# neobotix/neo_mpc_planner2

Measured on AMD Instinct MI355X. Metric: MPC solves/sec (control_steps=3, 500x500 costmap), higher is better.
Workload: dtype f64

## Files before the change

### neo_mpc_planner2_amd/csrc/adjoint.h

```cpp
#pragma once
#include "neo_mpc_device.h"
#include "wave_ops.h"
#include "fast_math.h"
#include "solver_context.h"
#include "costmap.h"
#include "riccati.h"

namespace neo_mpc {
namespace {

template <bool kTame, bool kRiccati, int kFew = 0>
__device__ __forceinline__ void adjoint_by_scans(const SolveArgs& a, const Ctx& c, double* L, bool exact_step, int lane, int n,
                                                 bool& free_path, int& nhops) {
  auto scan = [](double v) { if constexpr (kFew > 0) return wave_scan_few<kFew>(v); else return wave_scan(v); };
  constexpr int kLast = kFew > 0 ? kFew - 1 : 63;
  const DevParams& p = a.p;
  const double* u = L + a.lds.u;
  double* gs = L + a.lds.gs;
  float* RS = reinterpret_cast<float*>(L + a.lds.ric);
  float* ARTF = reinterpret_cast<float*>(L + a.lds.rt);
  const bool on = lane < n;
  const double vx = on ? u[3 * lane] : 0.0, vy = on ? u[3 * lane + 1] : 0.0, w = on ? u[3 * lane + 2] : 0.0;
  const double th = scan(w * p.dt);
  double sn, cs;
  sincos_heading<kTame>(th, &sn, &cs);
  const double ddx = (vx * cs - vy * sn) * p.dt, ddy = (vx * sn + vy * cs) * p.dt;
  const double x = scan(ddx), y = scan(ddy);
  double rt = on ? -2.0 * p.wo_n * (c.tyaw - th) : 0.0;
  if (lane == n - 1) rt += -2.0 * p.wterm_o * (c.fyaw - th);
  const double rx = on ? -2.0 * p.wt_n * (c.cx - x) : 0.0, ry = on ? -2.0 * p.wt_n * (c.cy - y) : 0.0;
  const double px = scan(rx), py = scan(ry);
  const double SX = lane_value(px, kLast) - px + rx, SY = lane_value(py, kLast) - py + ry;
  const double tt = on ? rt - ddy * SX + ddx * SY : 0.0;
  const double pt = scan(tt);
  const double ST = lane_value(pt, kLast) - pt + tt;
  int raw_here = 0;
  bool has_hop = false;
  float hop_x = 0.0f, hop_y = 0.0f;
  if (on) {
    gs[3 * lane] = p.dt * (cs * SX + sn * SY);
    gs[3 * lane + 1] = p.dt * (-sn * SX + cs * SY);
    gs[3 * lane + 2] = p.dt * ST;
    if (kRiccati) {
      float* rs = RS + kRicStage * lane;
      rs[RS_CS] = (float)cs; rs[RS_SN] = (float)sn; rs[RS_PX] = (float)ddx; rs[RS_PY] = (float)ddy;
      double wxx, wxy, wyy, wlx, wly;
      raw_here = edge_stickiness(a, c, L, x, y, cs, sn, wxx, wxy, wyy, wlx, wly, has_hop, hop_x, hop_y);
      rs[RS_WXX] = (float)wxx; rs[RS_WXY] = (float)wxy; rs[RS_WYY] = (float)wyy;
      rs[RS_WLX] = (float)wlx; rs[RS_WLY] = (float)wly;
      rs[RS_SY] = exact_step ? (float)SY : 0.0f;
      ARTF[2 * lane + 1] = exact_step ? (float)SX : 0.0f;
    }
  }
  if (kRiccati) {
    free_path = __ballot(raw_here != 0) == 0ull;
    const unsigned long long hmask = __ballot(has_hop);
    const int rank = __popcll(hmask & ((1ull << lane) - 1ull));
    double* t = L + a.lds.tol;
    if (has_hop && rank < kHopLanes) {
      reinterpret_cast<int*>(t + T_HOP_STAGE)[rank] = lane;
      reinterpret_cast<float*>(t + T_HOP_VEC)[2 * rank] = hop_x;
      reinterpret_cast<float*>(t + T_HOP_VEC)[2 * rank + 1] = hop_y;
    }
    nhops = min(__popcll(hmask), (int)kHopLanes);
    if (lane == 0) reinterpret_cast<int*>(t + T_HOP_STAGE)[kHopLanes] = nhops;
  }
  WAVE_SYNC();
}

template <int kSteps, bool kTame>
__device__ __forceinline__ void adjoint_short_sweep(const SolveArgs& a, const Ctx& c, double* L, bool have_trig, int lane, int n) {
  const DevParams& p = a.p;
  const double* u = L + a.lds.u;
  double* gs = L + a.lds.gs;
  double* ACS = L + a.lds.cs;
  double* ASN = L + a.lds.sn;
  double* ADX = L + a.lds.dxs;
  double* ADY = L + a.lds.dys;
  double* ARX = L + a.lds.rx;
  double* ARY = L + a.lds.ry;
// ... 36 lines not shown
```

### neo_mpc_planner2_amd/csrc/k1_solve.h

```cpp
#pragma once
#include <hip/hip_runtime.h>
#include <hip/hip_ext.h>
#include <math.h>
#include <stdint.h>
#include <stdlib.h>

#include "neo_mpc_device.h"
#include "wave_ops.h"
#include "fast_math.h"
#include "solver_context.h"
#include "solver_rules.h"
#include "costmap.h"
#include "feasible_set.h"
#include "rollout.h"
#include "riccati.h"
#include "adjoint.h"
#include "tangent_cone.h"
#include "dense_newton.h"
#include "lbfgs.h"
#include "cell_scan.h"
#include "k1_timing.h"

namespace neo_mpc {
namespace {

constexpr int kStallIterations = NEO_RULE_STALL_ITERATIONS;
constexpr int kBlockedRun = NEO_RULE_BLOCKED_RUN;
constexpr double kBlockedStep = NEO_RULE_BLOCKED_STEP;
constexpr double kFinalFracGaussNewton = NEO_RULE_FINAL_FRAC_GN;
// ... 143 lines not shown
  }
  s.flags = flags; s.cold = cold;
  return true;
}

template <int kMinWavesPerSimd, int kSteps, int kDir, bool kTame, int kStaticTile, int kLayoutSteps, bool kRouted = false>
__device__ __forceinline__ bool solve_search(double* L, uint32_t b, SolveCarry& sc) {
  constexpr bool kCovered = kStaticTile > 0;
  constexpr bool kNewton = kDir == 1;
  constexpr bool kRiccati = kDir == 2;
  constexpr bool kSecond = kDir != 0;
  constexpr bool kBlockedRule = kNewton || kRouted;
  static_assert(!kRiccati || kSteps == 0 || kRouted, "the stage-wise direction: run-time-sized, or the routed kernel's control_steps-3 branch");
  static_assert(!kRouted || (kRiccati && kSteps == kRoutedSteps), "the routed branch is the stage-wise one, three stages in registers");
  constexpr int kFew = (kRiccati && kSteps > 0) ? kSteps : 0;
  constexpr int kNwSteps = !kNewton ? 1 : kSteps ? kSteps : kNewtonMaxSteps;
  constexpr bool kVectorPose = kTame;
  constexpr int kRegSteps = kSteps ? kSteps : 1;
  constexpr int kPairs = kSteps ? 4 : NEO_MPC_MAX_LBFGS_MEMORY;
  double f = sc.f;
  const bool cold = sc.cold;
  int npairs = 0, head = 0, nfev = sc.nfev, it = sc.it, status = sc.status, stall = 0;
  int blocked_run = 0;
  int nblocked = 1;
  double u_term = 0.0;
  double gain1 = INFINITY, gain2 = INFINITY;
  bool final_step = false;
  double alpha = 1.0;
  bool scanned = false;
  int nscans = 0;
// ... 35 lines not shown
    if (kRouted && lane == 0) L[a.lds.tol + T_KINK] = p.kink_radius_stagewise;
    alpha = kRiccati ? fmax(1.0, n * 0.125) : 1.0;
    if (kFew && lane == 0) { double* t = L + a.lds.tol; t[T_GAIN1] = INFINITY; t[T_GAIN2] = INFINITY; t[T_ALPHA] = alpha; }
    if (kRiccati && lane == 0) L[a.lds.tol + T_MU] = n > 8 ? (double)(n - 8) * 0.125 : 0.0;
  }
  bool v_feasible = false;
  if (kRiccati) {
    double b0 = c.v0, b1 = c.v1, b2 = c.v2;
    asm volatile("" : "+v"(b0), "+v"(b1), "+v"(b2));
    project_block<kTame>(p, b0, b1, b2);
    v_feasible = b0 == c.v0 && b1 == c.v1 && b2 == c.v2;
  }
  double my_scale;
  {
    int l0 = lane_again();
    my_scale = kRiccati ? 0.0 : lane_scale<kSecond>(l0);
  }
  for (; it < p.max_it && !scan_only; ++it) {
    int lane = lane_again();
    const bool exact_step = kRiccati && nblocked == 0;
    int tol_off = a.lds.tol;
    asm volatile("" : "+s"(tol_off));
    const double* TOL = L + tol_off;
    NEO_PHASE_DECL;
    NEO_PHASE(0);
    constexpr int kVars = 3 * kNwSteps;
    const int nvr = kSteps ? kVars : nv;
    bool free_path = false;
    int nhops = 0;
    float hc[kVars];
    float newton_sol = 0.0f;
    if (kNewton) {
      double hcol[kSteps ? kVars : 1];
      const double hstep = 1e-6, inv_h = 1.0 / hstep;
      double pcs[kNwSteps], psn[kNwSteps];
      double x = 0.0, y = 0.0, th = 0.0;
    #pragma unroll
      for (int i = 0; i < kNwSteps; ++i) {
        if (kSteps || i < n) {
          const double vx = u[3 * i] + (lane == 3 * i ? hstep : 0.0);
          const double vy = u[3 * i + 1] + (lane == 3 * i + 1 ? hstep : 0.0);
          const double w = u[3 * i + 2] + (lane == 3 * i + 2 ? hstep : 0.0);
          th += w * p.dt;
          sincos_heading<kTame>(th, &psn[i], &pcs[i]);
          x += (vx * pcs[i] - vy * psn[i]) * p.dt;
          y += (vx * psn[i] + vy * pcs[i]) * p.dt;
// ... 25 lines not shown
          x -= pdx; y -= pdy; th -= w * p.dt;
        } else {
          hc[3 * k] = 0.0f; hc[3 * k + 1] = 0.0f; hc[3 * k + 2] = 0.0f;
        }
      }
      if (kSteps) {
    #pragma unroll
        for (int j = 0; j < kVars; ++j) {
          const double base = lane_value(hcol[j], 63);
          if (lane == 63) gs[j] = base;
          hc[j] = (float)((hcol[j] - base) * inv_h);
        }
      }
      WAVE_SYNC();
    }
    else if (!kSteps || kRiccati) adjoint_by_scans<kTame, kRiccati, kFew>(a, c, L, exact_step, lane, n, free_path, nhops);
    else adjoint_short_sweep<kSteps, kTame>(a, c, L, have_trig, lane, n);
    NEO_PHASE(1);
    const bool my_corner = tangent_cone_pass<kTame, kNewton, kRiccati>(a, c, L, TOL[T_KINK], lane, n);
    WAVE_SYNC();
    const bool corner_any = kSecond && !kTame && __ballot(my_corner) != 0ull && (kRiccati ? free_path : (it > 0 && u_term == 0.0));
    NEO_PHASE(2);
    if (p.max_it == kDumpGradient) {
      for (int k = lane; k < nv; k += kLanes) a.solution[(size_t)b * nv + k] = gt[k];
      return true;
    }
    if (kSecond && it == 0 && cold) {
      if (kRiccati) { for (int k = lane; k < nv; k += kLanes) d[k] = -gr[k]; }
      else if (lane < nvr) d[lane] = -gr[lane];
      if (kRiccati) for (int i = lane; i < n; i += kLanes) AMODE[4 * i + 3] = 0;
      WAVE_SYNC();
    } else if (kRiccati) {
      riccati_prepare(a, c, L, n, lane, v_feasible, (float)TOL[T_MU]);
      WAVE_SYNC();
      if (corner_any) riccati_keep_linear_terms(a, L, n, lane, true);
      auto sweep = [&]() {
        riccati_sweep<float, (kMinWavesPerSimd < 4), kFew>(a, L, n, lane);
        riccati_finish(a, c, L, n, lane);
      };
      sweep();
      if (!kTame && corner_any && repin_corner_blocks<true>(a, L, n, lane)) {
        riccati_keep_linear_terms(a, L, n, lane, false);
        sweep();
      }
    } else if (kNewton) {
      newton_sol = dense_newton_direction<kSteps, kNwSteps, kTame>(a, L, hc, corner_any, lane, n, nvr);
    }
    NEO_PHASE(3);
    if (!kSecond) lbfgs_direction<kSteps, kPairs>(a, L, it, mem, head, npairs, lane, n);
    if (kSecond && it > 0) {
      float dm = 0.0f;
      int anynear = 0;
      if (kRiccati) {
        for (int k = lane; k < nv; k += kLanes) {
          const float v = (float)fabs(d[k]);
          dm = (v == v) ? fmaxf(dm, v) : INFINITY;
          anynear |= (AMODE[4 * (k / 3) + 2] == 1);
        }
      } else if (lane < nvr) { dm = fabsf(newton_sol); anynear = (AMODE[4 * (lane / 3) + 2] == 1); }
      dm = wave_max_f(dm);
      const bool near_any = __ballot(anynear != 0) != 0ull;
      if ((double)dm < TOL[T_EARLY] && !near_any && nhops == 0) { status = NEO_MPC_STATUS_CONVERGED; break; }
      if ((double)dm < ((kRiccati && !exact_step) ? kFinalFracGaussNewton : 1.0) * TOL[T_FINAL] && !near_any) final_step = true;
    }
    NEO_PHASE(4);
    if (p.max_it > kDumpGradient && it == p.max_it - kDumpGradient - 1) {
      for (int k = lane; k < nv; k += kLanes) a.solution[(size_t)b * nv + k] = d[k];
      return true;
    }
    const double lscale = kRiccati ? lane_scale<kSecond>(lane) : my_scale;
    const double alpha_now = kFew ? TOL[T_ALPHA] : alpha;
    const double pstep = alpha_now * lscale;
    const double step = lane < 32 ? pstep : lscale;
    bool took_trial = false;
    double fb = INFINITY, cterm = 0.0;
    int best = 32;
    if (kRiccati && free_path && it > 0) took_trial = riccati_free_space_trial<kTame, kCovered, kFew, kBlockedRule>(a, c, L, n, lane, alpha_now, f, fb, cterm);
    const double* ALT0 = L + a.lds.state + S_PREV_U0;
    bool alt_armed = false;
    if (it == 0) alt_armed = uniform_int(reinterpret_cast<const int*>(L + a.lds.state)[SI_HAS_PREV]) == kAltArmed;
    if (!took_trial) {
    int hop_stage = -1;
    float hop_x = 0.0f, hop_y = 0.0f;
    if (kRiccati && lane >= 1 && lane <= nhops) {
      const double* t = TOL;
// ... 59 lines not shown
          candidate_block<kTame, kRiccati>(a, c, L, best, bstep, bpstep, i, b0, b1, b2, bhop, bhx, bhy);
          if (alt_won) { const double* src = i == 0 ? ALT0 : u + 3 * (i - 1); b0 = src[0]; b1 = src[1]; b2 = src[2]; }
          u_new[3 * i] = b0; u_new[3 * i + 1] = b1; u_new[3 * i + 2] = b2;
        }
      }
      have_trig = true;
      WAVE_SYNC();
      for (int k = lane; k < nv; k += kLanes) {
        const double nu = u_new[k], ou = u[k];
        stepmax = fmaxf(stepmax, (float)fabs(nu - ou));
        if (!kSecond) { u_prev[k] = ou; gt_prev[k] = gt[k]; }
        u[k] = nu;
      }
      stepmax = wave_max_f(stepmax);
    }
    const double gain = f - fb;
    const double fscale = fmax(1.0, fabs(fb));
    stall = (gain <= TOL[T_FTOL] * fscale || (double)stepmax <= TOL[T_STALL]) ? stall + 1 : 0;
    const bool hop_won = (kRiccati && best >= 1 && best <= nhops) || alt_won;
    nblocked = (best < 32 || lane_value(step, best) < kWindowStep || hop_won) ? nblocked + 1 : 0;
    const bool window_on = !kRiccati || kRouted || nblocked >= 3;
    const double wtol0 = TOL[T_WTOL];
    const double wtol = it >= kLateIteration ? TOL[T_WTOL_LATE] : wtol0;
    const double g1 = kFew ? TOL[T_GAIN1] : gain1, g2 = kFew ? TOL[T_GAIN2] : gain2;
    bool creeping = wtol > 0.0 && gain + g1 + g2 <= wtol * fscale && window_on;
    bool free_now = kRiccati ? free_path : false;
    if (kNewton) free_now = lane_value(cterm, best) == 0.0;
    creeping = creeping || (wtol0 > 0.0 && (double)stepmax <= TOL[T_STALL] && gain <= 0.5 * g1 && g1 <= 0.5 * g2 &&
                            (!free_now || (g2 < INFINITY && gain * gain <= TOL[T_FTOL] * fscale * (g1 - gain))) &&
                            ((kRiccati && !kRouted) ? window_on : nblocked >= kClosingRun));
    bool blocked_stop = false;
    if (kBlockedRule) {
      const double bs = lane_value(step, best);
      blocked_run = (best < 32 || bs < kBlockedStep) ? blocked_run + 1 : 0;
      if (blocked_run >= kBlockedRun) {
        const bool free_rollout = lane_value(cterm, best) == 0.0;
        const double btol = free_rollout ? TOL[T_BTOL_FREE] : TOL[T_BTOL_MAP];
        blocked_stop = gain + g1 + g2 <= btol;
      }
    }
    double* TOLW = L + tol_off;
    if (kFew) { if (lane == 0) { TOLW[T_GAIN2] = g1; TOLW[T_GAIN1] = gain; } }
    else { gain2 = gain1; gain1 = gain; }
    f = fb;
    if (nblocked != 0) final_step = false;
    if (kNewton) u_term = lane_value(cterm, best);
    if (kRiccati && !(it == 0 && cold) && !hop_won) {
      constexpr unsigned long long kNearlyFull = newton_lanes_at_least(0.8), kShort = kNewtonLanes & ~newton_lanes_at_least(0.3);
      const double mu0 = n > 8 ? (double)(n - 8) * 0.125 : 0.0, mu = TOL[T_MU];
      double* mu_slot = L + tol_off + T_MU;
      if ((kNearlyFull >> best) & 1ull) { if (lane == 0) *mu_slot = fmax(0.25 * mu, mu0 * 0.0625); }
      else if (best < 32 || ((kShort >> best) & 1ull)) { if (lane == 0) *mu_slot = fmin(4.0 * mu, 16.0 * mu0); }
    }
    if (best < 32 && !hop_won) {
      const double al = clampd(lane_value(step, best), 1e-6, 1e6);
      if (kFew) { if (lane == 0) TOLW[T_ALPHA] = al; }
      else alpha = al;
    }
    WAVE_SYNC();
    NEO_PHASE(6);
    NEO_PHASE_DUMP();
    if ((double)stepmax < TOL[T_XTOL] || stall >= kStallIterations || creeping || final_step || blocked_stop) { status = NEO_MPC_STATUS_CONVERGED; ++it; break; }
  }

  if (!kSecond || scanned || status != NEO_MPC_STATUS_CONVERGED || p.max_it >= kDumpGradient) break;
  const bool nothing_to_scan = (c.tile_geom & kTileFree) || (kNewton && u_term == 0.0);
  if (nothing_to_scan && nscans == 0) break;
  bool resume = false;
  {
    SolveArgs as;
    fresh_args<kSteps, kStaticTile, kLayoutSteps, kRouted>(as);
    select_map(as.map, L + as.lds.prob);
    Ctx cs;
    ctx_from_lds<false>(as, L, cs);
    int ls = lane_again();
    if (nscans == 0 && ls == 0) L[as.lds.tol + T_FSCAN] = f;
    NEO_SEGMENT_SCAN_BEGIN();
// ... 109 lines not shown
```

### neo_mpc_planner2_amd/csrc/riccati.h

```cpp
#pragma once
#include <hip/hip_runtime.h>
#include <math.h>
#include <stdint.h>

#include "neo_mpc_device.h"
#include "wave_ops.h"
#include "fast_math.h"
#include "solver_context.h"
#include "solver_rules.h"
#include "costmap.h"
#include "feasible_set.h"

namespace neo_mpc {
namespace {

enum : int {
  RS_PX = 0, RS_PY, RS_TX, RS_TY,
  RS_WXX, RS_WXY, RS_WYY, RS_FLAGS,
  RS_C00, RS_C01, RS_C02, RS_C11,
  RS_C12, RS_C22, RS_CS, RS_SN,
  RS_GT = 16,
  RS_GS = 19,
  RS_WK = 22,
  RS_WLX = 25, RS_WLY,
  RS_SY = 27,
  RS_GAIN = 16,
  kRicStage = 28
};
enum : int { RC_FREE3 = 0, RC_SLIDE_W, RC_XY, RC_SLIDE, RC_W, RC_NONE, RC_KINK, RF_CASE = 7, RF_KINK_OK = 8 };

typedef float ric_f4 __attribute__((ext_vector_type(4)));

__device__ __forceinline__ float ric_rcp(float x) { return __builtin_amdgcn_rcpf(x); }
__device__ __forceinline__ double ric_rcp(double x) { return rcp_fast(x); }
template <typename T> __device__ __forceinline__ T ric_max(T a, T b) { return a > b ? a : b; }
template <typename T> __device__ __forceinline__ T ric_abs(T a) { return a < (T)0 ? -a : a; }
__device__ __forceinline__ float ric_fma(float a, float b, float c) { return fmaf(a, b, c); }
__device__ __forceinline__ double ric_fma(double a, double b, double c) { return fma(a, b, c); }
template <typename T> __device__ __forceinline__ T ric_pivot(T p, T delta) { return p > delta ? p : ric_max(ric_abs(p), delta); }

__device__ __forceinline__ void riccati_prepare(const SolveArgs& a, const Ctx& c, double* L, int n, int lane,
                                                bool v_feasible, float mu) {
  if (lane >= n) return;
  const DevParams& p = a.p;
  float* rs = reinterpret_cast<float*>(L + a.lds.ric) + kRicStage * lane;
  const int* am = reinterpret_cast<const int*>(L + a.lds.mode) + 4 * lane;
  const double* gt = L + a.lds.gt + 3 * lane;
  const double* gs = L + a.lds.gs + 3 * lane;
  const double* u = L + a.lds.u + 3 * lane;
  const double cs = rs[RS_CS], sn = rs[RS_SN];
  const double idt = rcp_fast(p.dt);
  rs[RS_GT] = (float)((cs * gt[0] - sn * gt[1]) * idt); rs[RS_GT + 1] = (float)((sn * gt[0] + cs * gt[1]) * idt);
  rs[RS_GT + 2] = (float)(gt[2] * idt);
  rs[RS_GS] = (float)((cs * gs[0] - sn * gs[1]) * idt); rs[RS_GS + 1] = (float)((sn * gs[0] + cs * gs[1]) * idt);
  rs[RS_GS + 2] = (float)(gs[2] * idt);
  const double e0 = u[0] - c.v0, e1 = u[1] - c.v1, e2 = u[2] - c.v2;
  rs[RS_WK] = (float)(-(cs * e0 - sn * e1) * p.dt); rs[RS_WK + 1] = (float)(-(sn * e0 + cs * e1) * p.dt);
  rs[RS_WK + 2] = (float)(-e2 * p.dt);
  const double nx = L[a.lds.nx + lane], ny = L[a.lds.ny + lane];
  const double tx = -ny, ty = nx;
  const float rtx = (float)(cs * tx - sn * ty), rty = (float)(sn * tx + cs * ty);
  rs[RS_TX] = rtx; rs[RS_TY] = rty;
  const int near = am[2];
  const int xy = near ? 2 : am[0];
  const bool wfree = !(near || (am[1] & 1));
  const int kase = xy == 0 ? (wfree ? RC_FREE3 : RC_XY) : xy == 1 ? (wfree ? RC_SLIDE_W : RC_SLIDE) : (wfree ? RC_W : RC_NONE);
  const int flags = kase | ((!near && v_feasible) ? RF_KINK_OK : 0);
  rs[RS_FLAGS] = (float)flags;
  float c00 = 0.0f, c01 = 0.0f, c02 = 0.0f, c11 = 0.0f, c12 = 0.0f, c22 = 0.0f;
  if (!near) {
    const float f0 = (float)(cs * e0 - sn * e1), f1 = (float)(sn * e0 + cs * e1), f2 = (float)e2;
    const float fn2 = f0 * f0 + f1 * f1 + f2 * f2;
    const float ine = fn2 > 0.0f ? __builtin_amdgcn_rsqf(fn2) : 0.0f;
    const float i2 = (float)(idt * idt);
    const float sN = (float)p.wc_n * ine * i2, h0 = f0 * ine, h1 = f1 * ine, h2 = f2 * ine;
    const float k2 = reinterpret_cast<const float*>(L + a.lds.rt)[2 * lane] * i2;
    c00 = sN * (1.0f - h0 * h0) + k2 * rtx * rtx; c01 = -sN * h0 * h1 + k2 * rtx * rty; c02 = -sN * h0 * h2;
    c11 = sN * (1.0f - h1 * h1) + k2 * rty * rty; c12 = -sN * h1 * h2; c22 = sN * (1.0f - h2 * h2);
    const float mt = mu * (float)(2.0 * p.wt_n);
    c00 += mt; c11 += mt; c22 += mu * (float)(2.0 * p.wo_n);
  }
  rs[RS_C00] = c00; rs[RS_C01] = c01; rs[RS_C02] = c02; rs[RS_C11] = c11; rs[RS_C12] = c12; rs[RS_C22] = c22;
}

__device__ __forceinline__ void riccati_keep_linear_terms(const SolveArgs& a, double* L, int n, int lane, bool save) {
  ric_f4* rec = reinterpret_cast<ric_f4*>(reinterpret_cast<float*>(L + a.lds.ric) + kRicStage * lane + RS_GAIN);
  ric_f4* keep = reinterpret_cast<ric_f4*>(L + a.lds.keep) + 3 * lane;
  for (int i = lane; i < n; i += kLanes, rec += 7 * kLanes, keep += 3 * kLanes) {
    if (save) { keep[0] = rec[0]; keep[1] = rec[1]; keep[2] = rec[2]; }
    else { rec[0] = keep[0]; rec[1] = keep[1]; rec[2] = keep[2]; }
  }
  WAVE_SYNC();
}

template <typename T, bool kPrefetch = true, int kFew = 0>
__device__ __forceinline__ void riccati_sweep(const SolveArgs& a, double* L, int n, int lane) {
  const DevParams& p = a.p;
  float* RS = static_cast<float*>(__builtin_assume_aligned(reinterpret_cast<float*>(L + a.lds.ric), 16));
  int* AMODE = reinterpret_cast<int*>(L + a.lds.mode);
  double* d = L + a.lds.d;
  const float* ARTF = reinterpret_cast<const float*>(L + a.lds.rt);
  const T w2 = (T)(2.0 * p.wt_n), wo2 = (T)(2.0 * p.wo_n), wterm2 = (T)(2.0 * p.wterm_o);
  const T wc2 = (T)((p.wc_n * p.wc_n) / (p.dt * p.dt));

  T V00 = (T)0.0, V01 = (T)0.0, V02 = (T)0.0, V11 = (T)0.0, V12 = (T)0.0, V22 = (T)0.0, v0 = (T)0.0, v1 = (T)0.0, v2 = (T)0.0;
  ric_f4 r0, r1, r2, r3, r4, r5, r6;
  if (kPrefetch) {
    const ric_f4* R4 = reinterpret_cast<const ric_f4*>(RS + kRicStage * (n - 1));
    r0 = R4[0]; r1 = R4[1]; r2 = R4[2]; r3 = R4[3]; r4 = R4[4]; r5 = R4[5]; r6 = R4[6];
  }
  for (int i = (kFew ? kFew : n) - 1; i >= 0; --i) {
    const bool first = kFew > 0 && i == 0;
    if (!kPrefetch) {
      const ric_f4* R4 = reinterpret_cast<const ric_f4*>(RS + kRicStage * i);
      r0 = R4[0]; r1 = R4[1]; r2 = R4[2]; r3 = R4[3]; r4 = R4[4]; r5 = R4[5]; r6 = R4[6];
    }
    const T px = r0.x, py = r0.y, rtx = r0.z, rty = r0.w;
    const T wxx = r1.x, wxy = r1.y, wyy = r1.z;
    const int flags = __builtin_amdgcn_readfirstlane((int)r1.w);
    const T c00 = r2.x, c01 = r2.y, c02 = r2.z, c11 = r2.w, c12 = r3.x, c22 = r3.y;
    const T gt0 = r4.x, gt1 = r4.y, gt2 = r4.z, gs0 = r4.w, gs1 = r5.x, gs2 = r5.y, e0 = r5.z, e1 = r5.w, e2 = r6.x;
    v0 += (T)r6.y; v1 += (T)r6.z;
    const T sy = (T)r6.w, sx = (T)ARTF[2 * i + 1];
    if (kPrefetch && i > 0) {
      const ric_f4* R4 = reinterpret_cast<const ric_f4*>(RS + kRicStage * (i - 1));
      r0 = R4[0]; r1 = R4[1]; r2 = R4[2]; r3 = R4[3]; r4 = R4[4]; r5 = R4[5]; r6 = R4[6];
    }
    const T S00 = V00 + w2 + wxx, S01 = V01 + wxy, S11 = V11 + w2 + wyy;
    const T S22 = V22 + wo2 + (i == n - 1 ? wterm2 : (T)0.0);
    const T M02 = ric_fma(-py, S00, ric_fma(px, S01, V02));
// ... 119 lines not shown
        v2 = z2 + Z02 * k0 + Z12 * k1 + Z22 * k2;
        V00 = S00; V01 = S01; V02 = M02; V11 = S11; V12 = M12; V22 = Z22;
        break;
      default:
        v0 = z0; v1 = z1; v2 = z2;
        V00 = S00; V01 = S01; V02 = M02; V11 = S11; V12 = M12; V22 = Z22;
        break;
    }
    if (lane == 0) {
      ric_f4* G4 = reinterpret_cast<ric_f4*>(RS + kRicStage * i + RS_GAIN);
      G4[0] = ric_f4{(float)K00, (float)K01, (float)K02, (float)K10};
      G4[1] = ric_f4{(float)K11, (float)K12, (float)K20, (float)K21};
      G4[2] = ric_f4{(float)K22, (float)k0, (float)k1, (float)k2};
      AMODE[4 * i + 3] = tokink ? 1 : 0;
    }
  }
  WAVE_SYNC();
  T z0 = (T)0.0, z1 = (T)0.0, z2 = (T)0.0;
  for (int i = 0; i < n; ++i) {
    const ric_f4* R4 = reinterpret_cast<const ric_f4*>(RS + kRicStage * i);
    const ric_f4 s0 = R4[0], g0 = R4[4], g1 = R4[5], g2 = R4[6];
    const T w0 = (T)g2.y + (T)g0.x * z0 + (T)g0.y * z1 + (T)g0.z * z2;
    const T w1 = (T)g2.z + (T)g0.w * z0 + (T)g1.x * z1 + (T)g1.y * z2;
    const T w2f = (T)g2.w + (T)g1.z * z0 + (T)g1.w * z1 + (T)g2.x * z2;
    if (lane == 0) { d[3 * i] = (double)w0; d[3 * i + 1] = (double)w1; d[3 * i + 2] = (double)w2f; }
    const T e0 = z0 + w0, e1 = z1 + w1, e2 = z2 + w2f;
    z0 = ric_fma(-(T)s0.y, e2, e0); z1 = ric_fma((T)s0.x, e2, e1); z2 = e2;
  }
  WAVE_SYNC();
}

__device__ __forceinline__ void riccati_finish(const SolveArgs& a, const Ctx& c, double* L, int n, int lane) {
  if (lane < n) {
    const float* rs = reinterpret_cast<const float*>(L + a.lds.ric) + kRicStage * lane;
    const int* am = reinterpret_cast<const int*>(L + a.lds.mode) + 4 * lane;
    double* d = L + a.lds.d + 3 * lane;
    if (am[3]) {
      const double* u = L + a.lds.u + 3 * lane;
      d[0] = c.v0 - u[0]; d[1] = c.v1 - u[1]; d[2] = c.v2 - u[2];
    } else {
      const double cs = rs[RS_CS], sn = rs[RS_SN], idt = rcp_fast(a.p.dt);
      const double w0 = d[0], w1 = d[1], w2 = d[2];
      double d0 = (cs * w0 + sn * w1) * idt, d1 = (-sn * w0 + cs * w1) * idt;
      const int mode = am[2] ? 2 : am[0];
      if (mode == 1) {
        const double nx = L[a.lds.nx + lane], ny = L[a.lds.ny + lane];
        const double dot = d0 * nx + d1 * ny;
        d0 -= dot * nx; d1 -= dot * ny;
      } else if (mode == 2) { d0 = 0.0; d1 = 0.0; }
      d[0] = d0; d[1] = d1; d[2] = (am[2] || (am[1] & 1)) ? 0.0 : w2 * idt;
    }
  }
  WAVE_SYNC();
}

template <bool kTame, bool kCovered, int kFew, bool kWantTerm>
__device__ __forceinline__ bool riccati_free_space_trial(const SolveArgs& a, const Ctx& c, double* L, int n, int lane,
// ... 40 lines not shown
```

### neo_mpc_planner2_amd/csrc/tangent_cone.h

```cpp
#pragma once
#include "neo_mpc_device.h"
#include "fast_math.h"
#include "solver_context.h"
#include "solver_rules.h"
#include "riccati.h"

namespace neo_mpc {
namespace {

constexpr int kNewtonRecord = 13;

template <bool kTame, bool kNewton, bool kRiccati>
__device__ __forceinline__ bool tangent_cone_pass(const SolveArgs& a, const Ctx& c, double* L, double kink_radius, int lane, int n) {
  constexpr bool kSecond = kNewton || kRiccati;
  const DevParams& p = a.p;
  const double* u = L + a.lds.u;
  double* gs = L + a.lds.gs;
  double* gt = L + a.lds.gt;
  double* gr = L + a.lds.gr;
  double* ANX = L + a.lds.nx;
  double* ANY = L + a.lds.ny;
  int* AMODE = reinterpret_cast<int*>(L + a.lds.mode);
  float* NB = reinterpret_cast<float*>(L + a.lds.cs);
  float* ARTF = reinterpret_cast<float*>(L + a.lds.rt);
  bool my_corner = false;
  for (int i = lane; i < n; i += kLanes) {
    const double u0 = u[3 * i], u1 = u[3 * i + 1], u2 = u[3 * i + 2];
    const double g0 = gs[3 * i], g1 = gs[3 * i + 1], g2 = gs[3 * i + 2];
    const double e0 = u0 - c.v0, e1 = u1 - c.v1, e2 = u2 - c.v2;
    const double ne2 = e0 * e0 + e1 * e1 + e2 * e2;
    const double ine = ne2 > 0.0 ? rsq_fast(ne2) : 0.0;
    const double ne = ne2 * ine;
    double t0, t1, t2;
    if (ne2 > 0.0) {
      const double wn = p.wc_n * ine;
      t0 = g0 + wn * e0; t1 = g1 + wn * e1; t2 = g2 + wn * e2;
    } else {
      const double ng2 = g0 * g0 + g1 * g1 + g2 * g2;
      const double sh = (ng2 > p.wc_n * p.wc_n) ? 1.0 - p.wc_n * rsq_fast(ng2) : 0.0;
      t0 = g0 * sh; t1 = g1 * sh; t2 = g2 * sh;
    }
    if (!kRiccati) AMODE[4 * i + 3] = AMODE[4 * i + 2];
    const bool near = ne < kink_radius;
// ... 35 lines not shown
#undef NEO_TRY_SLIDE
      if (mode == 2) { r0 = 0.0; r1 = 0.0; }
    }
    if (near) {
      const double s2 = wfroz ? 0.0 : t2;
      gs[3 * i] = r0; gs[3 * i + 1] = r1; gs[3 * i + 2] = s2;
      gt[3 * i] = 0.0; gt[3 * i + 1] = 0.0; gt[3 * i + 2] = 0.0;
      gr[3 * i] = 0.0; gr[3 * i + 1] = 0.0; gr[3 * i + 2] = 0.0;
      const int at_rest = (ne2 == 0.0 && r0 * r0 + r1 * r1 + s2 * s2 <= p.wc_n * p.wc_n) ? 2 : 1;
      ANX[i] = 0.0; ANY[i] = 0.0; AMODE[4 * i] = 0; AMODE[4 * i + 1] = 0; AMODE[4 * i + 2] = at_rest;
      if (kNewton) {
#pragma unroll
        for (int k = 0; k < kNewtonRecord; ++k) NB[kNewtonRecord * i + k] = 0.0f;
      }
      if (kRiccati) ARTF[2 * i] = 0.0f;
      continue;
    }
    gr[3 * i] = r0; gr[3 * i + 1] = r1; gr[3 * i + 2] = wfroz ? 0.0 : t2;
    if (kSecond && !kTame && !p.disc_in_box && mode == 1) {
      const double room = NEO_RULE_CORNER_ROOM, rin = p.r - room;
      my_corner = my_corner || (mslot != 0 && (u0 - p.lo[0] <= room || p.hi[0] - u0 <= room)) ||
                  (mslot != 1 && (u1 - p.lo[1] <= room || p.hi[1] - u1 <= room)) || (mslot != 2 && nvv2 >= rin * rin);
    }
    ANX[i] = mnx; ANY[i] = mny; AMODE[4 * i] = mode; AMODE[4 * i + 1] = wfroz | ((mode == 1 && mslot == 2) ? 2 : 0); AMODE[4 * i + 2] = 0;
    if (kNewton) {
      float* nb = NB + kNewtonRecord * i;
      nb[0] = mode == 0 ? 1.0f : mode == 1 ? (float)(1.0 - mnx * mnx) : 0.0f;
      nb[1] = mode == 1 ? (float)(-mnx * mny) : 0.0f;
      nb[2] = mode == 0 ? 1.0f : mode == 1 ? (float)(1.0 - mny * mny) : 0.0f;
      nb[3] = wfroz ? 0.0f : 1.0f;
      const float f0 = (float)e0, f1 = (float)e1, f2 = (float)e2;
      const float fn2 = f0 * f0 + f1 * f1 + f2 * f2;
      const float ine = fn2 > 0.0f ? __builtin_amdgcn_rsqf(fn2) : 0.0f;
      const float sN = (float)p.wc_n * ine, h0 = f0 * ine, h1 = f1 * ine, h2 = f2 * ine;
      const float k2 = (mode == 1 && mslot == 2) ? (float)(mlam * rcp_fast(p.r)) : 0.0f;
      const float tx = -(float)mny, ty = (float)mnx;
      const float c00 = sN * (1.0f - h0 * h0) + k2 * tx * tx, c01 = -sN * h0 * h1 + k2 * tx * ty,
                  c02 = -sN * h0 * h2, c11 = sN * (1.0f - h1 * h1) + k2 * ty * ty, c12 = -sN * h1 * h2,
                  c22 = sN * (1.0f - h2 * h2);
      nb[4] = c00; nb[5] = c01; nb[6] = c02;
      nb[7] = c01; nb[8] = c11; nb[9] = c12;
      nb[10] = c02; nb[11] = c12; nb[12] = c22;
    }
    if (kRiccati) ARTF[2 * i] = (mode == 1 && mslot == 2) ? (float)(mlam * rcp_fast(p.r)) : 0.0f;
  }
  return my_corner;
}

template <bool kRiccati>
__device__ __forceinline__ bool repin_corner_blocks(const SolveArgs& a, double* L, int n, int lane) {
  int* AMODE = reinterpret_cast<int*>(L + a.lds.mode);
  const double* d = L + a.lds.d;
  const double* u = L + a.lds.u;
  double* gr = L + a.lds.gr;
  const DevParams& p = a.p;
  bool any = false;
  for (int i = lane; i < n; i += kLanes) {
    int* am = AMODE + 4 * i;
    if (am[0] != 1 || (kRiccati && am[3])) continue;
// ... 29 lines not shown
```

Measured before the change: 24.62 million.

## Forward per-stage solver state in registers across adjoint, cone and Riccati passes

Adds a StageRegs struct that carries each lane's stage data (controls, gradients, trig, cone normals, modes, Riccati outputs) in registers from the adjoint scan through the tangent-cone pass, Riccati prepare, sweep and finish. This replaces LDS round-trips, drops several wave barriers, caches tolerance values in registers, and lets the sweep load only the head of the next stage record ahead of time. It applies only to the routed three-step tame Riccati path. The cost is more live registers, which could reduce occupancy, and more code paths that must keep the LDS and register copies consistent.

```diff
diff --git a/neo_mpc_planner2_amd/csrc/adjoint.h b/neo_mpc_planner2_amd/csrc/adjoint.h
--- a/neo_mpc_planner2_amd/csrc/adjoint.h
+++ b/neo_mpc_planner2_amd/csrc/adjoint.h
@@ -5,13 +5,14 @@
 #include "solver_context.h"
 #include "costmap.h"
 #include "riccati.h"
+#include "stagewise3.h"
 
 namespace neo_mpc {
 namespace {
 
-template <bool kTame, bool kRiccati, int kFew = 0>
+template <bool kTame, bool kRiccati, int kFew = 0, bool kForward = false>
 __device__ __forceinline__ void adjoint_by_scans(const SolveArgs& a, const Ctx& c, double* L, bool exact_step, int lane, int n,
-                                                 bool& free_path, int& nhops) {
+                                                 bool& free_path, int& nhops, StageRegs* fw = nullptr) {
   auto scan = [](double v) { if constexpr (kFew > 0) return wave_scan_few<kFew>(v); else return wave_scan(v); };
   constexpr int kLast = kFew > 0 ? kFew - 1 : 63;
   const DevParams& p = a.p;
@@ -37,10 +38,12 @@
   int raw_here = 0;
   bool has_hop = false;
   float hop_x = 0.0f, hop_y = 0.0f;
+  double g0 = 0.0, g1 = 0.0, g2 = 0.0;
   if (on) {
-    gs[3 * lane] = p.dt * (cs * SX + sn * SY);
-    gs[3 * lane + 1] = p.dt * (-sn * SX + cs * SY);
-    gs[3 * lane + 2] = p.dt * ST;
+    g0 = p.dt * (cs * SX + sn * SY);
+    g1 = p.dt * (-sn * SX + cs * SY);
+    g2 = p.dt * ST;
+    gs[3 * lane] = g0; gs[3 * lane + 1] = g1; gs[3 * lane + 2] = g2;
     if (kRiccati) {
       float* rs = RS + kRicStage * lane;
       rs[RS_CS] = (float)cs; rs[RS_SN] = (float)sn; rs[RS_PX] = (float)ddx; rs[RS_PY] = (float)ddy;
@@ -64,6 +67,12 @@
     }
     nhops = min(__popcll(hmask), (int)kHopLanes);
     if (lane == 0) reinterpret_cast<int*>(t + T_HOP_STAGE)[kHopLanes] = nhops;
+  }
+  if (kForward) {
+    fw->u0 = vx; fw->u1 = vy; fw->u2 = w; fw->g0 = g0; fw->g1 = g1; fw->g2 = g2; fw->cs = (float)cs; fw->sn = (float)sn;
+    fw_keep(fw->u0); fw_keep(fw->u1); fw_keep(fw->u2); fw_keep(fw->g0); fw_keep(fw->g1); fw_keep(fw->g2);
+    fw_keep(fw->cs); fw_keep(fw->sn);
+    return;
   }
   WAVE_SYNC();
 }
diff --git a/neo_mpc_planner2_amd/csrc/k1_solve.h b/neo_mpc_planner2_amd/csrc/k1_solve.h
--- a/neo_mpc_planner2_amd/csrc/k1_solve.h
+++ b/neo_mpc_planner2_amd/csrc/k1_solve.h
@@ -13,6 +13,7 @@
 #include "costmap.h"
 #include "feasible_set.h"
 #include "rollout.h"
+#include "stagewise3.h"
 #include "riccati.h"
 #include "adjoint.h"
 #include "tangent_cone.h"
@@ -186,6 +187,7 @@
   static_assert(!kRiccati || kSteps == 0 || kRouted, "the stage-wise direction: run-time-sized, or the routed kernel's control_steps-3 branch");
   static_assert(!kRouted || (kRiccati && kSteps == kRoutedSteps), "the routed branch is the stage-wise one, three stages in registers");
   constexpr int kFew = (kRiccati && kSteps > 0) ? kSteps : 0;
+  constexpr bool kForward = kFew > 0 && kTame;
   constexpr int kNwSteps = !kNewton ? 1 : kSteps ? kSteps : kNewtonMaxSteps;
   constexpr bool kVectorPose = kTame;
   constexpr int kRegSteps = kSteps ? kSteps : 1;
@@ -251,7 +253,7 @@
   double my_scale;
   {
     int l0 = lane_again();
-    my_scale = kRiccati ? 0.0 : lane_scale<kSecond>(l0);
+    my_scale = (kRiccati && !kForward) ? 0.0 : lane_scale<kSecond>(l0);
   }
   for (; it < p.max_it && !scan_only; ++it) {
     int lane = lane_again();
@@ -259,6 +261,9 @@
     int tol_off = a.lds.tol;
     asm volatile("" : "+s"(tol_off));
     const double* TOL = L + tol_off;
+    double tb[kTolDoubles];
+    if (kForward) { tb[T_KINK] = TOL[T_KINK]; tb[T_MU] = TOL[T_MU]; }
+    auto tol = [&](int k) { return kForward ? tb[k] : TOL[k]; };
     NEO_PHASE_DECL;
     NEO_PHASE(0);
     constexpr int kVars = 3 * kNwSteps;
@@ -267,6 +272,7 @@
     int nhops = 0;
     float hc[kVars];
     float newton_sol = 0.0f;
+    StageRegs fw = {};
     if (kNewton) {
       double hcol[kSteps ? kVars : 1];
       const double hstep = 1e-6, inv_h = 1.0 / hstep;
@@ -322,31 +328,35 @@
       }
       WAVE_SYNC();
     }
-    else if (!kSteps || kRiccati) adjoint_by_scans<kTame, kRiccati, kFew>(a, c, L, exact_step, lane, n, free_path, nhops);
+    else if (!kSteps || kRiccati) adjoint_by_scans<kTame, kRiccati, kFew, kForward>(a, c, L, exact_step, lane, n, free_path, nhops, &fw);
     else adjoint_short_sweep<kSteps, kTame>(a, c, L, have_trig, lane, n);
     NEO_PHASE(1);
-    const bool my_corner = tangent_cone_pass<kTame, kNewton, kRiccati>(a, c, L, TOL[T_KINK], lane, n);
-    WAVE_SYNC();
+    const bool my_corner = tangent_cone_pass<kTame, kNewton, kRiccati, kForward>(a, c, L, tol(T_KINK), lane, n, &fw);
+    if (!kForward) WAVE_SYNC();
     const bool corner_any = kSecond && !kTame && __ballot(my_corner) != 0ull && (kRiccati ? free_path : (it > 0 && u_term == 0.0));
     NEO_PHASE(2);
     if (p.max_it == kDumpGradient) {
+      if (kForward) WAVE_SYNC();
       for (int k = lane; k < nv; k += kLanes) a.solution[(size_t)b * nv + k] = gt[k];
       return true;
     }
     if (kSecond && it == 0 && cold) {
+      if (kForward) WAVE_SYNC();
       if (kRiccati) { for (int k = lane; k < nv; k += kLanes) d[k] = -gr[k]; }
       else if (lane < nvr) d[lane] = -gr[lane];
       if (kRiccati) for (int i = lane; i < n; i += kLanes) AMODE[4 * i + 3] = 0;
       WAVE_SYNC();
     } else if (kRiccati) {
-      riccati_prepare(a, c, L, n, lane, v_feasible, (float)TOL[T_MU]);
+      riccati_prepare<kForward>(a, c, L, n, lane, v_feasible, (float)tol(T_MU), &fw);
+      if (kForward) fw.face = stage_face(fw.mode, fw.wfroz, fw.near);
       WAVE_SYNC();
       if (corner_any) riccati_keep_linear_terms(a, L, n, lane, true);
       auto sweep = [&]() {
-        riccati_sweep<float, (kMinWavesPerSimd < 4), kFew>(a, L, n, lane);
-        riccati_finish(a, c, L, n, lane);
+        riccati_sweep<float, (kMinWavesPerSimd < 4), kFew, kForward, (kForward && kMinWavesPerSimd >= 4)>(a, L, n, lane, &fw);
+        riccati_finish<kForward>(a, c, L, n, lane, &fw);
       };
       sweep();
+      static_assert(!kForward || kTame, "a re-pin changes a block's face in LDS: the forwarded copy (StageRegs::face) would be stale");
       if (!kTame && corner_any && repin_corner_blocks<true>(a, L, n, lane)) {
         riccati_keep_linear_terms(a, L, n, lane, false);
         sweep();
@@ -376,7 +386,7 @@
       for (int k = lane; k < nv; k += kLanes) a.solution[(size_t)b * nv + k] = d[k];
       return true;
     }
-    const double lscale = kRiccati ? lane_scale<kSecond>(lane) : my_scale;
+    const double lscale = (kRiccati && !kForward) ? lane_scale<kSecond>(lane) : my_scale;
     const double alpha_now = kFew ? TOL[T_ALPHA] : alpha;
     const double pstep = alpha_now * lscale;
     const double step = lane < 32 ? pstep : lscale;
@@ -466,20 +476,25 @@
       }
       stepmax = wave_max_f(stepmax);
     }
+    if (kForward) {
+      tb[T_FTOL] = TOL[T_FTOL]; tb[T_STALL] = TOL[T_STALL]; tb[T_WTOL] = TOL[T_WTOL]; tb[T_WTOL_LATE] = TOL[T_WTOL_LATE];
+      tb[T_GAIN1] = TOL[T_GAIN1]; tb[T_GAIN2] = TOL[T_GAIN2]; tb[T_BTOL_FREE] = TOL[T_BTOL_FREE]; tb[T_BTOL_MAP] = TOL[T_BTOL_MAP];
+      tb[T_MU] = TOL[T_MU]; tb[T_XTOL] = TOL[T_XTOL];
+    }
     const double gain = f - fb;
     const double fscale = fmax(1.0, fabs(fb));
-    stall = (gain <= TOL[T_FTOL] * fscale || (double)stepmax <= TOL[T_STALL]) ? stall + 1 : 0;
+    stall = (gain <= tol(T_FTOL) * fscale || (double)stepmax <= tol(T_STALL)) ? stall + 1 : 0;
     const bool hop_won = (kRiccati && best >= 1 && best <= nhops) || alt_won;
     nblocked = (best < 32 || lane_value(step, best) < kWindowStep || hop_won) ? nblocked + 1 : 0;
     const bool window_on = !kRiccati || kRouted || nblocked >= 3;
-    const double wtol0 = TOL[T_WTOL];
-    const double wtol = it >= kLateIteration ? TOL[T_WTOL_LATE] : wtol0;
-    const double g1 = kFew ? TOL[T_GAIN1] : gain1, g2 = kFew ? TOL[T_GAIN2] : gain2;
+    const double wtol0 = tol(T_WTOL);
+    const double wtol = it >= kLateIteration ? tol(T_WTOL_LATE) : wtol0;
+    const double g1 = kFew ? tol(T_GAIN1) : gain1, g2 = kFew ? tol(T_GAIN2) : gain2;
     bool creeping = wtol > 0.0 && gain + g1 + g2 <= wtol * fscale && window_on;
     bool free_now = kRiccati ? free_path : false;
     if (kNewton) free_now = lane_value(cterm, best) == 0.0;
-    creeping = creeping || (wtol0 > 0.0 && (double)stepmax <= TOL[T_STALL] && gain <= 0.5 * g1 && g1 <= 0.5 * g2 &&
-                            (!free_now || (g2 < INFINITY && gain * gain <= TOL[T_FTOL] * fscale * (g1 - gain))) &&
+    creeping = creeping || (wtol0 > 0.0 && (double)stepmax <= tol(T_STALL) && gain <= 0.5 * g1 && g1 <= 0.5 * g2 &&
+                            (!free_now || (g2 < INFINITY && gain * gain <= tol(T_FTOL) * fscale * (g1 - gain))) &&
                             ((kRiccati && !kRouted) ? window_on : nblocked >= kClosingRun));
     bool blocked_stop = false;
     if (kBlockedRule) {
@@ -487,7 +502,7 @@
       blocked_run = (best < 32 || bs < kBlockedStep) ? blocked_run + 1 : 0;
       if (blocked_run >= kBlockedRun) {
         const bool free_rollout = lane_value(cterm, best) == 0.0;
-        const double btol = free_rollout ? TOL[T_BTOL_FREE] : TOL[T_BTOL_MAP];
+        const double btol = free_rollout ? tol(T_BTOL_FREE) : tol(T_BTOL_MAP);
         blocked_stop = gain + g1 + g2 <= btol;
       }
     }
@@ -499,7 +514,7 @@
     if (kNewton) u_term = lane_value(cterm, best);
     if (kRiccati && !(it == 0 && cold) && !hop_won) {
       constexpr unsigned long long kNearlyFull = newton_lanes_at_least(0.8), kShort = kNewtonLanes & ~newton_lanes_at_least(0.3);
-      const double mu0 = n > 8 ? (double)(n - 8) * 0.125 : 0.0, mu = TOL[T_MU];
+      const double mu0 = n > 8 ? (double)(n - 8) * 0.125 : 0.0, mu = tol(T_MU);
       double* mu_slot = L + tol_off + T_MU;
       if ((kNearlyFull >> best) & 1ull) { if (lane == 0) *mu_slot = fmax(0.25 * mu, mu0 * 0.0625); }
       else if (best < 32 || ((kShort >> best) & 1ull)) { if (lane == 0) *mu_slot = fmin(4.0 * mu, 16.0 * mu0); }
@@ -512,7 +527,7 @@
     WAVE_SYNC();
     NEO_PHASE(6);
     NEO_PHASE_DUMP();
-    if ((double)stepmax < TOL[T_XTOL] || stall >= kStallIterations || creeping || final_step || blocked_stop) { status = NEO_MPC_STATUS_CONVERGED; ++it; break; }
+    if ((double)stepmax < tol(T_XTOL) || stall >= kStallIterations || creeping || final_step || blocked_stop) { status = NEO_MPC_STATUS_CONVERGED; ++it; break; }
   }
 
   if (!kSecond || scanned || status != NEO_MPC_STATUS_CONVERGED || p.max_it >= kDumpGradient) break;
diff --git a/neo_mpc_planner2_amd/csrc/riccati.h b/neo_mpc_planner2_amd/csrc/riccati.h
--- a/neo_mpc_planner2_amd/csrc/riccati.h
+++ b/neo_mpc_planner2_amd/csrc/riccati.h
@@ -10,6 +10,7 @@
 #include "solver_rules.h"
 #include "costmap.h"
 #include "feasible_set.h"
+#include "stagewise3.h"
 
 namespace neo_mpc {
 namespace {
@@ -39,16 +40,20 @@
 __device__ __forceinline__ double ric_fma(double a, double b, double c) { return fma(a, b, c); }
 template <typename T> __device__ __forceinline__ T ric_pivot(T p, T delta) { return p > delta ? p : ric_max(ric_abs(p), delta); }
 
+template <bool kForward = false>
 __device__ __forceinline__ void riccati_prepare(const SolveArgs& a, const Ctx& c, double* L, int n, int lane,
-                                                bool v_feasible, float mu) {
+                                                bool v_feasible, float mu, const StageRegs* fw = nullptr) {
   if (lane >= n) return;
   const DevParams& p = a.p;
   float* rs = reinterpret_cast<float*>(L + a.lds.ric) + kRicStage * lane;
   const int* am = reinterpret_cast<const int*>(L + a.lds.mode) + 4 * lane;
-  const double* gt = L + a.lds.gt + 3 * lane;
-  const double* gs = L + a.lds.gs + 3 * lane;
-  const double* u = L + a.lds.u + 3 * lane;
-  const double cs = rs[RS_CS], sn = rs[RS_SN];
+  const double* gtl = L + a.lds.gt + 3 * lane;
+  const double* gsl = L + a.lds.gs + 3 * lane;
+  const double* ul = L + a.lds.u + 3 * lane;
+  const double gt[3] = {kForward ? fw->t0 : gtl[0], kForward ? fw->t1 : gtl[1], kForward ? fw->t2 : gtl[2]};
+  const double gs[3] = {kForward ? fw->g0 : gsl[0], kForward ? fw->g1 : gsl[1], kForward ? fw->g2 : gsl[2]};
+  const double u[3] = {kForward ? fw->u0 : ul[0], kForward ? fw->u1 : ul[1], kForward ? fw->u2 : ul[2]};
+  const double cs = kForward ? fw->cs : rs[RS_CS], sn = kForward ? fw->sn : rs[RS_SN];
   const double idt = rcp_fast(p.dt);
   rs[RS_GT] = (float)((cs * gt[0] - sn * gt[1]) * idt); rs[RS_GT + 1] = (float)((sn * gt[0] + cs * gt[1]) * idt);
   rs[RS_GT + 2] = (float)(gt[2] * idt);
@@ -57,13 +62,13 @@
   const double e0 = u[0] - c.v0, e1 = u[1] - c.v1, e2 = u[2] - c.v2;
   rs[RS_WK] = (float)(-(cs * e0 - sn * e1) * p.dt); rs[RS_WK + 1] = (float)(-(sn * e0 + cs * e1) * p.dt);
   rs[RS_WK + 2] = (float)(-e2 * p.dt);
-  const double nx = L[a.lds.nx + lane], ny = L[a.lds.ny + lane];
+  const double nx = kForward ? fw->nx : L[a.lds.nx + lane], ny = kForward ? fw->ny : L[a.lds.ny + lane];
   const double tx = -ny, ty = nx;
   const float rtx = (float)(cs * tx - sn * ty), rty = (float)(sn * tx + cs * ty);
   rs[RS_TX] = rtx; rs[RS_TY] = rty;
-  const int near = am[2];
-  const int xy = near ? 2 : am[0];
-  const bool wfree = !(near || (am[1] & 1));
+  const int near = kForward ? fw->near : am[2];
+  const int xy = near ? 2 : (kForward ? fw->mode : am[0]);
+  const bool wfree = !(near || ((kForward ? fw->wfroz : am[1]) & 1));
   const int kase = xy == 0 ? (wfree ? RC_FREE3 : RC_XY) : xy == 1 ? (wfree ? RC_SLIDE_W : RC_SLIDE) : (wfree ? RC_W : RC_NONE);
   const int flags = kase | ((!near && v_feasible) ? RF_KINK_OK : 0);
   rs[RS_FLAGS] = (float)flags;
@@ -74,7 +79,7 @@
     const float ine = fn2 > 0.0f ? __builtin_amdgcn_rsqf(fn2) : 0.0f;
     const float i2 = (float)(idt * idt);
     const float sN = (float)p.wc_n * ine * i2, h0 = f0 * ine, h1 = f1 * ine, h2 = f2 * ine;
-    const float k2 = reinterpret_cast<const float*>(L + a.lds.rt)[2 * lane] * i2;
+    const float k2 = (kForward ? fw->k2 : reinterpret_cast<const float*>(L + a.lds.rt)[2 * lane]) * i2;
     c00 = sN * (1.0f - h0 * h0) + k2 * rtx * rtx; c01 = -sN * h0 * h1 + k2 * rtx * rty; c02 = -sN * h0 * h2;
     c11 = sN * (1.0f - h1 * h1) + k2 * rty * rty; c12 = -sN * h1 * h2; c22 = sN * (1.0f - h2 * h2);
     const float mt = mu * (float)(2.0 * p.wt_n);
@@ -93,8 +98,10 @@
   WAVE_SYNC();
 }
 
-template <typename T, bool kPrefetch = true, int kFew = 0>
-__device__ __forceinline__ void riccati_sweep(const SolveArgs& a, double* L, int n, int lane) {
+template <typename T, bool kPrefetch = true, int kFew = 0, bool kForward = false, bool kHead = false>
+__device__ __forceinline__ void riccati_sweep(const SolveArgs& a, double* L, int n, int lane, StageRegs* fw = nullptr) {
+  static_assert(!(kPrefetch && kHead), "the whole record or its head");
+  static_assert(kRicStage % 4 == 0, "a stage record is a whole number of 16-byte words");
   const DevParams& p = a.p;
   float* RS = static_cast<float*>(__builtin_assume_aligned(reinterpret_cast<float*>(L + a.lds.ric), 16));
   int* AMODE = reinterpret_cast<int*>(L + a.lds.mode);
@@ -109,11 +116,18 @@
     const ric_f4* R4 = reinterpret_cast<const ric_f4*>(RS + kRicStage * (n - 1));
     r0 = R4[0]; r1 = R4[1]; r2 = R4[2]; r3 = R4[3]; r4 = R4[4]; r5 = R4[5]; r6 = R4[6];
   }
+  ric_f4 h0, h1;
+  if (kHead) {
+    const ric_f4* R4 = reinterpret_cast<const ric_f4*>(RS + kRicStage * ((kFew ? kFew : n) - 1));
+    h0 = R4[0]; h1 = R4[1];
+  }
   for (int i = (kFew ? kFew : n) - 1; i >= 0; --i) {
     const bool first = kFew > 0 && i == 0;
     if (!kPrefetch) {
       const ric_f4* R4 = reinterpret_cast<const ric_f4*>(RS + kRicStage * i);
-      r0 = R4[0]; r1 = R4[1]; r2 = R4[2]; r3 = R4[3]; r4 = R4[4]; r5 = R4[5]; r6 = R4[6];
+      if (kHead) { r0 = h0; r1 = h1; } else { r0 = R4[0]; r1 = R4[1]; }
+      r2 = R4[2]; r3 = R4[3]; r4 = R4[4]; r5 = R4[5]; r6 = R4[6];
+      if (kHead && i > 0) { h0 = R4[-(kRicStage / 4)]; h1 = R4[1 - kRicStage / 4]; }
     }
     const T px = r0.x, py = r0.y, rtx = r0.z, rty = r0.w;
     const T wxx = r1.x, wxy = r1.y, wyy = r1.z;
@@ -263,6 +277,7 @@
       G4[2] = ric_f4{(float)K22, (float)k0, (float)k1, (float)k2};
       AMODE[4 * i + 3] = tokink ? 1 : 0;
     }
+    if (kForward && lane == i) fw->tokink = tokink ? 1 : 0;
   }
   WAVE_SYNC();
   T z0 = (T)0.0, z1 = (T)0.0, z2 = (T)0.0;
@@ -272,24 +287,29 @@
     const T w0 = (T)g2.y + (T)g0.x * z0 + (T)g0.y * z1 + (T)g0.z * z2;
     const T w1 = (T)g2.z + (T)g0.w * z0 + (T)g1.x * z1 + (T)g1.y * z2;
     const T w2f = (T)g2.w + (T)g1.z * z0 + (T)g1.w * z1 + (T)g2.x * z2;
-    if (lane == 0) { d[3 * i] = (double)w0; d[3 * i + 1] = (double)w1; d[3 * i + 2] = (double)w2f; }
+    if (kForward) { if (lane == i) { fw->w0 = (double)w0; fw->w1 = (double)w1; fw->w2 = (double)w2f; } }
+    else if (lane == 0) { d[3 * i] = (double)w0; d[3 * i + 1] = (double)w1; d[3 * i + 2] = (double)w2f; }
     const T e0 = z0 + w0, e1 = z1 + w1, e2 = z2 + w2f;
     z0 = ric_fma(-(T)s0.y, e2, e0); z1 = ric_fma((T)s0.x, e2, e1); z2 = e2;
   }
-  WAVE_SYNC();
-}
-
-__device__ __forceinline__ void riccati_finish(const SolveArgs& a, const Ctx& c, double* L, int n, int lane) {
+  if (kForward) { fw_keep(fw->w0); fw_keep(fw->w1); fw_keep(fw->w2); fw_keep(fw->tokink); return; }
+  WAVE_SYNC();
+}
+
+template <bool kForward = false>
+__device__ __forceinline__ void riccati_finish(const SolveArgs& a, const Ctx& c, double* L, int n, int lane, const StageRegs* fw = nullptr) {
   if (lane < n) {
     const float* rs = reinterpret_cast<const float*>(L + a.lds.ric) + kRicStage * lane;
-    const int* am = reinterpret_cast<const int*>(L + a.lds.mode) + 4 * lane;
+    const int* aml = reinterpret_cast<const int*>(L + a.lds.mode) + 4 * lane;
+    const int am[4] = {kForward ? (fw->face & 3) : aml[0], kForward ? ((fw->face >> 2) & 1) : aml[1], kForward ? 0 : aml[2],
+                       kForward ? fw->tokink : aml[3]};
     double* d = L + a.lds.d + 3 * lane;
     if (am[3]) {
       const double* u = L + a.lds.u + 3 * lane;
       d[0] = c.v0 - u[0]; d[1] = c.v1 - u[1]; d[2] = c.v2 - u[2];
     } else {
-      const double cs = rs[RS_CS], sn = rs[RS_SN], idt = rcp_fast(a.p.dt);
-      const double w0 = d[0], w1 = d[1], w2 = d[2];
+      const double cs = kForward ? fw->cs : rs[RS_CS], sn = kForward ? fw->sn : rs[RS_SN], idt = rcp_fast(a.p.dt);
+      const double w0 = kForward ? fw->w0 : d[0], w1 = kForward ? fw->w1 : d[1], w2 = kForward ? fw->w2 : d[2];
       double d0 = (cs * w0 + sn * w1) * idt, d1 = (-sn * w0 + cs * w1) * idt;
       const int mode = am[2] ? 2 : am[0];
       if (mode == 1) {
diff --git a/neo_mpc_planner2_amd/csrc/stagewise3.h b/neo_mpc_planner2_amd/csrc/stagewise3.h
--- /dev/null
+++ b/neo_mpc_planner2_amd/csrc/stagewise3.h
@@ -0,0 +1,27 @@
+#pragma once
+#include <hip/hip_runtime.h>
+
+namespace neo_mpc {
+namespace {
+
+struct StageRegs {
+  double u0, u1, u2;
+  double g0, g1, g2;
+  double t0, t1, t2;
+  double nx, ny;
+  double w0, w1, w2;
+  float cs, sn;
+  float k2;
+  int mode, wfroz, near, tokink;
+  int face;
+};
+__device__ __forceinline__ int stage_face(int mode, int wfroz, int near) {
+  return (near ? 2 : mode) | ((near || (wfroz & 1)) ? 4 : 0);
+}
+
+__device__ __forceinline__ void fw_keep(double& v) { asm volatile("" : "+v"(v)); }
+__device__ __forceinline__ void fw_keep(float& v) { asm volatile("" : "+v"(v)); }
+__device__ __forceinline__ void fw_keep(int& v) { asm volatile("" : "+v"(v)); }
+
+}
+}
diff --git a/neo_mpc_planner2_amd/csrc/tangent_cone.h b/neo_mpc_planner2_amd/csrc/tangent_cone.h
--- a/neo_mpc_planner2_amd/csrc/tangent_cone.h
+++ b/neo_mpc_planner2_amd/csrc/tangent_cone.h
@@ -4,14 +4,16 @@
 #include "solver_context.h"
 #include "solver_rules.h"
 #include "riccati.h"
+#include "stagewise3.h"
 
 namespace neo_mpc {
 namespace {
 
 constexpr int kNewtonRecord = 13;
 
-template <bool kTame, bool kNewton, bool kRiccati>
-__device__ __forceinline__ bool tangent_cone_pass(const SolveArgs& a, const Ctx& c, double* L, double kink_radius, int lane, int n) {
+template <bool kTame, bool kNewton, bool kRiccati, bool kForward = false>
+__device__ __forceinline__ bool tangent_cone_pass(const SolveArgs& a, const Ctx& c, double* L, double kink_radius, int lane, int n,
+                                                  StageRegs* fw = nullptr) {
   constexpr bool kSecond = kNewton || kRiccati;
   const DevParams& p = a.p;
   const double* u = L + a.lds.u;
@@ -24,9 +26,9 @@
   float* NB = reinterpret_cast<float*>(L + a.lds.cs);
   float* ARTF = reinterpret_cast<float*>(L + a.lds.rt);
   bool my_corner = false;
-  for (int i = lane; i < n; i += kLanes) {
-    const double u0 = u[3 * i], u1 = u[3 * i + 1], u2 = u[3 * i + 2];
-    const double g0 = gs[3 * i], g1 = gs[3 * i + 1], g2 = gs[3 * i + 2];
+  auto block = [&](int i) __attribute__((always_inline)) {
+    const double u0 = kForward ? fw->u0 : u[3 * i], u1 = kForward ? fw->u1 : u[3 * i + 1], u2 = kForward ? fw->u2 : u[3 * i + 2];
+    const double g0 = kForward ? fw->g0 : gs[3 * i], g1 = kForward ? fw->g1 : gs[3 * i + 1], g2 = kForward ? fw->g2 : gs[3 * i + 2];
     const double e0 = u0 - c.v0, e1 = u1 - c.v1, e2 = u2 - c.v2;
     const double ne2 = e0 * e0 + e1 * e1 + e2 * e2;
     const double ine = ne2 > 0.0 ? rsq_fast(ne2) : 0.0;
@@ -92,7 +94,11 @@
         for (int k = 0; k < kNewtonRecord; ++k) NB[kNewtonRecord * i + k] = 0.0f;
       }
       if (kRiccati) ARTF[2 * i] = 0.0f;
-      continue;
+      if (kForward) {
+        fw->g0 = r0; fw->g1 = r1; fw->g2 = s2; fw->t0 = 0.0; fw->t1 = 0.0; fw->t2 = 0.0; fw->nx = 0.0; fw->ny = 0.0;
+        fw->k2 = 0.0f; fw->mode = 0; fw->wfroz = 0; fw->near = at_rest;
+      }
+      return;
     }
     gr[3 * i] = r0; gr[3 * i + 1] = r1; gr[3 * i + 2] = wfroz ? 0.0 : t2;
     if (kSecond && !kTame && !p.disc_in_box && mode == 1) {
@@ -100,7 +106,8 @@
       my_corner = my_corner || (mslot != 0 && (u0 - p.lo[0] <= room || p.hi[0] - u0 <= room)) ||
                   (mslot != 1 && (u1 - p.lo[1] <= room || p.hi[1] - u1 <= room)) || (mslot != 2 && nvv2 >= rin * rin);
     }
-    ANX[i] = mnx; ANY[i] = mny; AMODE[4 * i] = mode; AMODE[4 * i + 1] = wfroz | ((mode == 1 && mslot == 2) ? 2 : 0); AMODE[4 * i + 2] = 0;
+    const int wslot = wfroz | ((mode == 1 && mslot == 2) ? 2 : 0);
+    ANX[i] = mnx; ANY[i] = mny; AMODE[4 * i] = mode; AMODE[4 * i + 1] = wslot; AMODE[4 * i + 2] = 0;
     if (kNewton) {
       float* nb = NB + kNewtonRecord * i;
       nb[0] = mode == 0 ? 1.0f : mode == 1 ? (float)(1.0 - mnx * mnx) : 0.0f;
@@ -120,7 +127,18 @@
       nb[7] = c01; nb[8] = c11; nb[9] = c12;
       nb[10] = c02; nb[11] = c12; nb[12] = c22;
     }
-    if (kRiccati) ARTF[2 * i] = (mode == 1 && mslot == 2) ? (float)(mlam * rcp_fast(p.r)) : 0.0f;
+    const float disc_k2 = (kRiccati && mode == 1 && mslot == 2) ? (float)(mlam * rcp_fast(p.r)) : 0.0f;
+    if (kRiccati) ARTF[2 * i] = disc_k2;
+    if (kForward) {
+      fw->t0 = t0; fw->t1 = t1; fw->t2 = t2; fw->nx = mnx; fw->ny = mny;
+      fw->k2 = disc_k2; fw->mode = mode; fw->wfroz = wslot; fw->near = 0;
+    }
+  };
+  if constexpr (kForward) { if (lane < n) block(lane); }
+  else { for (int i = lane; i < n; i += kLanes) block(i); }
+  if (kForward) {
+    fw_keep(fw->g0); fw_keep(fw->g1); fw_keep(fw->g2); fw_keep(fw->t0); fw_keep(fw->t1); fw_keep(fw->t2);
+    fw_keep(fw->nx); fw_keep(fw->ny); fw_keep(fw->k2); fw_keep(fw->mode); fw_keep(fw->wfroz); fw_keep(fw->near);
   }
   return my_corner;
 }
```

Result: faster. 27.29 million (median of 6 runs) (+10.8%).
